# tyshiwo1/Accelerating-T2I-AR-with-SJD

Measured on AMD Instinct MI355X. Metric: accepted image-tokens/s (SJD, Lumina-mGPT-7B 768px); tokens_per_step = 1/steps-to-converge rate, higher is better.
Workload: dtype bf16; 1 GPU; Lumina-mGPT-7B 768x768, 1 prompt/GPU, draft window 16, CFG 3.0 (batch 2), top-k 2000, bf16, random-init synthetic weights (embed_token_scale=0.7); prompt_len=64, kv_len_start=401, kv_len_end=2064, lead_in_steps=131, prompts=1, parallelism=prompt-parallel x1

## Files before the change

### accelerating-t2i-ar-with-sjd_amd/_lib.py

```python
import ctypes
import os

MAX_WINDOW = 64
MAX_RANGES = 4
DTYPE_BF16, DTYPE_F16, DTYPE_F32 = 0, 1, 2
F1_POST_NORM = 0x100
F2_ROPE_TABLE = 0x200
QKN_SHARDS_SHIFT = 16

_HERE = os.path.dirname(os.path.abspath(__file__))
SO_PATH = os.environ.get("SJD_HIP_LIB") or os.path.join(_HERE, "libsjd_hip.so")


class RowRule(ctypes.Structure):
    _fields_ = [("n_ranges", ctypes.c_int32), ("lo", ctypes.c_int32 * MAX_RANGES), ("hi", ctypes.c_int32 * MAX_RANGES),
                ("forced", ctypes.c_int32), ("top_k", ctypes.c_int32), ("top_p_thr", ctypes.c_float), ("temperature", ctypes.c_float)]


class IterParams(ctypes.Structure):
    _fields_ = [("n_rows", ctypes.c_int32), ("kv_len", ctypes.c_int32), ("use_cfg", ctypes.c_int32),
                ("scheme", ctypes.c_int32), ("n_fresh", ctypes.c_int32), ("batch_rows", ctypes.c_int32), ("iter_seq", ctypes.c_int32), ("philox_blocks", ctypes.c_int32),
                ("philox_seed", ctypes.c_uint64), ("philox_offset", ctypes.c_uint64 * 3),
                ("fresh_tok", ctypes.c_int64 * MAX_WINDOW), ("rules", RowRule * MAX_WINDOW),
                ("resid_rules", RowRule * MAX_WINDOW)]


class State(ctypes.Structure):
    _fields_ = [("m", ctypes.c_int32), ("rejected", ctypes.c_int32), ("n_prev", ctypes.c_int32),
                ("prob_buf", ctypes.c_int32), ("tokens", ctypes.c_int64 * MAX_WINDOW),
                ("win_tok", ctypes.c_int64 * MAX_WINDOW), ("q_src", ctypes.c_int32 * MAX_WINDOW), ("amax", ctypes.c_int64 * MAX_WINDOW)]


class RowNorm(ctypes.Structure):
    _fields_ = [("sumsq", ctypes.c_void_p), ("slices", ctypes.c_int32), ("hidden", ctypes.c_int32), ("eps", ctypes.c_float)]


class Slots(ctypes.Structure):
    _fields_ = [("n_slots", ctypes.c_int32), ("head_rows", ctypes.c_int32), ("params_stride", ctypes.c_int64), ("state_stride", ctypes.c_int64),
                ("probs_stride", ctypes.c_int64), ("zero_state_stride", ctypes.c_int64), ("scratch_stride", ctypes.c_int64),
                ("mirror_stride", ctypes.c_int64), ("dbg_stride", ctypes.c_int64)]


class HeadPartials(ctypes.Structure):
    _fields_ = [("part", ctypes.c_void_p), ("n_chunks", ctypes.c_int32), ("chunk_stride", ctypes.c_int64), ("row_stride", ctypes.c_int64),
                ("col0", ctypes.c_int32), ("n_cols", ctypes.c_int32), ("urow_off", ctypes.c_int32), ("round_dtype", ctypes.c_int32),
                ("row_sumsq", ctypes.c_void_p), ("slices", ctypes.c_int32), ("prows", ctypes.c_int32), ("inv_hidden", ctypes.c_float),
                ("eps", ctypes.c_float), ("dbg_c", ctypes.c_void_p), ("dbg_u", ctypes.c_void_p), ("zero_state", ctypes.c_void_p)]


class L2Head(ctypes.Structure):
    _fields_ = [("wz", ctypes.c_void_p), ("kind", ctypes.c_int32), ("gx", ctypes.c_int32), ("gy", ctypes.c_int32), ("waves", ctypes.c_int32),
                ("n_tiles", ctypes.c_int32), ("tile0", ctypes.c_int32), ("n_out", ctypes.c_int32), ("pairs_full", ctypes.c_int32),
                ("pairs_last", ctypes.c_int32), ("step_major", ctypes.c_int32), ("head_pairs", ctypes.c_int32)]


EXPORTS = ["sjd_version", "sjd_error_string", "sjd_reguess", "sjd_logits_to_probs_sample", "sjd_verify_accept",
           "sjd_kv_append", "sjd_attention_workspace_bytes", "sjd_draft_window_attention", "sjd_draft_window_attention_ex",
# ... 135 lines not shown
```

### accelerating-t2i-ar-with-sjd_amd/backbones.py

```python
import math
from dataclasses import dataclass
from typing import Optional

import torch
import torch.nn as nn
import torch.nn.functional as F


import logging as _logging
import os as _os
_log = _logging.getLogger("sjd_amd.backbones")

_K1_FUSED_DEFAULT = _os.environ.get("SJD_K1_FUSED", "0") == "1"
_K1_FUSED_SPLIT_DEFAULT = _os.environ.get("SJD_K1_FUSED_SPLIT", "1") != "0"
_MLP_PAIR_DEFAULT = _os.environ.get("SJD_MLP_PAIR", "0") == "1"
_NAN_CHECK = _os.environ.get("SJD_NAN_CHECK", "0") == "1"


def _chk(tag, x, rows=None):
    if not _NAN_CHECK or x is None:
        return x
    t = x.data if hasattr(x, "n_chunks") else x
    v = t if rows is None else (t[:, :rows] if hasattr(x, "n_chunks") else t[:rows])
    if not torch.isfinite(v.float()).all():
# ... 590 lines not shown
        self.buffers_version = getattr(self, "buffers_version", 0) + 1
        return scales

    def _f2(self, qkv, li, qn, pos, B, n, params, kv_len, row_norm=None):
        ops, H, Hkv, D = self._ops, self.n_heads, self.n_kv_heads, self.head_dim
        return ops.qknorm_rope_append(qkv, self.cache.k[li], self.cache.v[li], *qn, self._inv_freq32, pos, B, n, H, Hkv, D, params,
                                      kv_len if params is None else 0, kv_scale=self.attn.scale_of(li) if hasattr(self.attn, "scale_of") else (1.0, 1.0),
                                      dtype=self.lm_head.weight.dtype, row_norm=row_norm, qk_shards=self.args.model_parallel_size)

    def _attention_block(self, qkv_part, li, qn, pos, B, n, params, kv_len, key_start, row_norm=None):
        ops, H, Hkv, D = self._ops, self.n_heads, self.n_kv_heads, self.head_dim
        ks_ok = isinstance(key_start, torch.Tensor) and key_start.is_cuda and key_start.dtype == torch.int32
        if getattr(self, "k1_fused", _K1_FUSED_DEFAULT) and ks_ok and not self.args.swin_norm and self.args.model_parallel_size == 1 and ops.fused_attention_ok(B, n, H, Hkv, D, self.cache.k.dtype):
            ns, ws = 1, None
            if getattr(self, "k1_fused_split", _K1_FUSED_SPLIT_DEFAULT):
                ns = self.attn._resolve_split(B, Hkv, n, H)
                ws = self.attn._workspace(B, H, n, D, self.cache.k.device) if ns > 1 else None
            return ops.qkv_attention_fused(qkv_part, self.cache.k[li], self.cache.v[li], *qn, self._inv_freq32, pos, B, n, H, D, params,
                                           kv_len if params is None else 0, key_start, row_norm=row_norm, dtype=self.lm_head.weight.dtype,
                                           n_split=ns, workspace=ws)
        q = self._f2(qkv_part, li, qn, pos, B, n, params, kv_len, row_norm=row_norm)
        return self.attn.attend(li, q, self.cache, kv_len, key_start)

    def _forward_window_g1_folded(self, tokens, positions, kv_len, key_start, cols=None, head_partials=False):
        ops, B, n = self._ops, tokens.shape[0], tokens.shape[1]
        T, eps, cfg = B * n, self.args.rms_norm_eps, self.G1_CFG
        self._prefetch_plan()
        g1 = lambda x_, name, N_, K_: self._g1(li, x_, name, N_, K_)
        H, Hkv, D, hid, inter = self.n_heads, self.n_kv_heads, self.head_dim, self.args.hidden_size, self.args.intermediate_size
        params = getattr(self.attn, "params", None)
        want_fused = getattr(self, "gateup_fused", _GATEUP_FUSED_DEFAULT)
        fuse_mlp = want_fused and (T <= 64 or want_fused == "tall") and not self._pf_on and ops.gateup_silu_ok(T, inter, hid, cfg["gate_up"][0],
                                                                                                                   isinstance(self._packed[0]["gate_up"], ops.PackedZ))
        red = getattr(self, "reduce_fused", _REDUCE_FUSED_DEFAULT) and not self._pf_on
        raw = lambda name: not isinstance(self._packed[0][name], ops.PackedZ)
        h_dev = self.lm_head.weight.device
        red_o = red and raw("o") and ops.skinny_gemm_reduce_ok(T, hid, H * D, cfg["o"][0], 8, h_dev)
        red_d = red and raw("down") and ops.skinny_gemm_reduce_ok(T, hid, inter, cfg["down"][0], 8, h_dev)
        pair_mlp = (getattr(self, "mlp_pair", _MLP_PAIR_DEFAULT) and fuse_mlp and not red_d and h_dev.type == "cuda" and
                    ops.mlp_pair_ok(T, inter, hid, self._packed[0]["gate_up"], self._packed[0]["down"], cfg["down"][0], cfg["down"][1], h_dev))
        h = self.model.embed_tokens(tokens).view(T, -1).contiguous()
        pos = positions.reshape(T).contiguous()
        delta, ss_next = None, None
        for li, layer in enumerate(self.model.layers):
            a = layer.self_attn
            rn = (ss_next if ss_next is not None else ops.residual_sumsq(h, delta), hid, eps)
            qn = (a.q_norm.weight, a.q_norm.bias, a.k_norm.weight, a.k_norm.bias) if self.args.qk_norm else (None,) * 4
            _chk(f"L{li} sumsq", rn[0][:, :T] if rn[0].dim() == 2 and rn[0].shape[1] >= T else rn[0])
            o = self._attention_block(_chk(f"L{li} qkv", g1(h, "qkv", (H + 2 * Hkv) * D, hid), T), li, qn, pos, B, n, params, kv_len, key_start, row_norm=rn)
            _chk(f"L{li} attention", o)
            if red_o:
                rn = (ops.skinny_gemm_reduce(o.view(T, H * D), self._packed[li]["o"], hid, H * D, cfg["o"][0], h, 8, cfg["o"][2]), hid, eps)
            else:
                rn = (ops.residual_sumsq(h, g1(o.view(T, H * D), "o", hid, H * D)), hid, eps)
            if pair_mlp:
                if getattr(self, "_pair_ready", None) is None or self._pair_ready.device != h.device:
                    self._pair_ready = torch.zeros(max(64, (inter + cfg["down"][0] - 1) // cfg["down"][0] + 1), dtype=torch.int32, device=h.device)
                _, delta = ops.mlp_pair(h, self._packed[li]["gate_up"], self._packed[li]["down"], inter, hid, cfg["down"][0], row_norm=rn,
                                        ready=self._pair_ready)
                ss_next = None
                continue
            if fuse_mlp:
                act = ops.gateup_silu(h, self._packed[li]["gate_up"], inter, hid, cfg["gate_up"][2], row_norm=rn)
            else:
                act = ops.silu_mul(g1(h, "gate_up", 2 * inter, hid), rows=T, dtype=h.dtype, row_norm=rn)
            _chk(f"L{li} act", act)
# ... 25 lines not shown
        pos = positions.reshape(T).contiguous()
        delta = None
        swin = self.args.swin_norm
        for li, layer in enumerate(self.model.layers):
            a = layer.self_attn
            x = h if swin else ops.add_rmsnorm(h, delta, layer.input_layernorm.weight, eps)
            qkv = g1(x, "qkv", (H + 2 * Hkv) * D, hid)
            qn = (a.q_norm.weight, a.q_norm.bias, a.k_norm.weight, a.k_norm.bias) if self.args.qk_norm else (None,) * 4
            o = self._attention_block(qkv, li, qn, pos, B, n, params, kv_len, key_start)
            attn_out = g1(o.view(T, H * D), "o", hid, H * D)
            if swin:
                x = ops.add_rmsnorm_post(h, attn_out, layer.input_layernorm.weight, eps)
            else:
                x = ops.add_rmsnorm(h, attn_out, layer.post_attention_layernorm.weight, eps)
            gu = g1(x, "gate_up", 2 * inter, hid)
            act = ops.silu_mul(gu, rows=T, dtype=h.dtype)
            delta = g1(act, "down", hid, inter)
            if swin:
                ops.add_rmsnorm_post(h, delta, layer.post_attention_layernorm.weight, eps)
                delta = None
        x = ops.add_rmsnorm(h, delta, self.model.norm.weight, eps)
        return _head_logits(self.lm_head, x, cols).view(B, n, -1)

    def _forward_window_fused(self, tokens, positions, kv_len, key_start, cols=None, head_partials=False):
        T_ = tokens.shape[0] * tokens.shape[1]
        if self._gemm == "sjd" and (T_ <= 64 or (T_ <= 128 and tokens.shape[1] <= 32) or
                                    (T_ <= 256 and tokens.shape[1] <= 32 and self._packed and not isinstance(self._packed[0]["qkv"], self._ops.PackedZ)
                                     and all(c[1] in self.G1_WIDE_TILES for c in self.G1_CFG.values()))):
            if self._fold_norm:
                return self._forward_window_g1_folded(tokens, positions, kv_len, key_start, cols, head_partials)
            return self._forward_window_g1(tokens, positions, kv_len, key_start, cols)
        ops, B, n = self._ops, tokens.shape[0], tokens.shape[1]
        T, eps = B * n, self.args.rms_norm_eps
        H, Hkv, D = self.n_heads, self.n_kv_heads, self.head_dim
        params = getattr(self.attn, "params", None)
        h = self.model.embed_tokens(tokens).view(T, -1).contiguous()
        pos = positions.reshape(T).contiguous()
        delta = None
        swin = self.args.swin_norm
        for li, layer in enumerate(self.model.layers):
            a = layer.self_attn
            qkv_w, gu_w = self._fused[li]
            x = h if swin else ops.add_rmsnorm(h, delta, layer.input_layernorm.weight, eps)
            qkv = F.linear(x, qkv_w)
            qn = (a.q_norm.weight, a.q_norm.bias, a.k_norm.weight, a.k_norm.bias) if self.args.qk_norm else (None,) * 4
            q = _chk(f"prefill L{li} q", self._f2(_chk(f"prefill L{li} qkv", qkv), li, qn, pos, B, n, params, kv_len))
            o = _chk(f"prefill L{li} attention", self.attn.attend(li, q, self.cache, kv_len, key_start))
            attn_out = F.linear(o.view(T, H * D), a.o_proj.weight)
            if swin:
                x = _chk(f"prefill L{li} norm1", ops.add_rmsnorm_post(h, attn_out, layer.input_layernorm.weight, eps))
                ops.add_rmsnorm_post(h, _chk(f"prefill L{li} mlp", F.linear(ops.silu_mul(F.linear(x, gu_w)), layer.mlp.down_proj.weight)),
                                     layer.post_attention_layernorm.weight, eps)
                continue
            x = _chk(f"prefill L{li} norm2", ops.add_rmsnorm(h, attn_out, layer.post_attention_layernorm.weight, eps))
            delta = _chk(f"prefill L{li} mlp", F.linear(ops.silu_mul(F.linear(x, gu_w)), layer.mlp.down_proj.weight))
        x = ops.add_rmsnorm(h, delta, self.model.norm.weight, eps)
        return _head_logits(self.lm_head, x, cols).view(B, n, -1)

    def forward_window(self, tokens, positions, kv_len, key_start, cols=None, head_partials=False):
        if getattr(self, "_ops", None) is not None:
            return self._forward_window_fused(tokens, positions, kv_len, key_start, cols, head_partials)
        B, n = tokens.shape
        h = self.model.embed_tokens(tokens)
        cos, sin = self._rope(positions, h.dtype)
        for li, layer in enumerate(self.model.layers):
            a = layer.self_attn
            x = h if self.args.swin_norm else layer.input_layernorm(h)
            q = a.q_proj(x).view(B, n, a.num_heads, a.head_dim)
            k = a.k_proj(x).view(B, n, a.num_kv, a.head_dim)
            v = a.v_proj(x).view(B, n, a.num_kv, a.head_dim)
            if self.args.qk_norm:
                q, k = a.q_norm(q), a.k_norm(k)
            q = q * cos + _rotate_half(q) * sin
            k = k * cos + _rotate_half(k) * sin
            o = self.attn(li, q, k, v, self.cache, kv_len, key_start)
            if self.args.swin_norm:
                h = h + layer.input_layernorm(a.o_proj(o.reshape(B, n, -1)))
                h = h + layer.post_attention_layernorm(layer.mlp(h))
                continue
            h = h + a.o_proj(o.reshape(B, n, -1))
            h = h + layer.mlp(layer.post_attention_layernorm(h))
        return _head_logits(self.lm_head, self.model.norm(h), cols)


# ... 8 lines not shown
```

### accelerating-t2i-ar-with-sjd_amd/csrc/sjd_glue.hip

```cpp
#include <hip/hip_runtime.h>
#include <math.h>

#include "../../include/sjd_hip.h"

#ifdef SJD_TRACE
__device__ unsigned long long g_glue_trace[3][4096][4];
#define SJD_TRG(k, i) do { if (threadIdx.x == 0) g_glue_trace[k][((blockIdx.y * gridDim.x) + blockIdx.x) & 4095][i] = wall_clock64(); } while (0)
extern "C" int sjd_debug_trace_glue(int kind, unsigned long long *host_out, int n_wg)
{
    return hipMemcpyFromSymbol(host_out, HIP_SYMBOL(g_glue_trace), (size_t)n_wg * 4 * sizeof(unsigned long long),
                               (size_t)kind * 4096 * 4 * sizeof(unsigned long long), hipMemcpyDeviceToHost) == hipSuccess ? 0 : -1;
}
#else
#define SJD_TRG(k, i) do { } while (0)
#endif

typedef __attribute__((ext_vector_type(4))) unsigned u32x4;

#include "sjd_mlp_epilogue.h"
#ifdef SJD_EXPERIMENTAL
#include "sjd_l2_prefetch.h"
#endif

template <int DT> struct Cvt;
template <> struct Cvt<SJD_DTYPE_BF16> {
    static __device__ __forceinline__ float to_f(unsigned short h) { return __uint_as_float((unsigned)h << 16); }
    static __device__ __forceinline__ unsigned short from_f(float x)
    {
        unsigned u = __float_as_uint(x);
        u += 0x7fffu + ((u >> 16) & 1u);
        return (unsigned short)(u >> 16);
    }
};
template <> struct Cvt<SJD_DTYPE_F16> {
    static __device__ __forceinline__ float to_f(unsigned short h) { return (float)(*reinterpret_cast<_Float16 *>(&h)); }
    static __device__ __forceinline__ unsigned short from_f(float x)
    {
        _Float16 h = (_Float16)x;
        return *reinterpret_cast<unsigned short *>(&h);
    }
};

// ... 225 lines not shown
            for (int j = 0; j < 4; ++j) {
                o[j] = sjd_residual_elem<DT>(hx[j], dd[j]);
                hx[j] = Cvt<DT>::to_f(o[j]);
            }
            uint2 ho;
            ho.x = (unsigned)o[0] | ((unsigned)o[1] << 16);
            ho.y = (unsigned)o[2] | ((unsigned)o[3] << 16);
            *reinterpret_cast<uint2 *>(hp) = ho;
        }
        ss = sjd_sumsq4(ss, hx[0], hx[1], hx[2], hx[3]);
    }
    ss = wave_sum(ss);
    if ((threadIdx.x & 63) == 0) red[threadIdx.x >> 6] = ss;
    __syncthreads();
    if (threadIdx.x == 0) out_sumsq[(size_t)blockIdx.y * prows + row] = red[0] + red[1];
    SJD_TRG(0, 2);
}

template <int DT>
__global__ __launch_bounds__(128) void f1r_residual_sumsq(unsigned short *__restrict__ h, const float *__restrict__ part, int n_chunks,
                                                          int hidden, int prows, float *__restrict__ out_sumsq)
{
    f1r_body<DT>(h, part, n_chunks, hidden, prows, out_sumsq);
}

#ifdef SJD_EXPERIMENTAL
template <int DT>
__global__ __launch_bounds__(128) void f1r_residual_sumsq_pf(unsigned short *__restrict__ h, const float *__restrict__ part, int n_chunks,
                                                             int hidden, int prows, float *__restrict__ out_sumsq, int n_slices,
                                                             const sjd_l2_head pf)
{
    if ((int)blockIdx.y >= n_slices) {
        sjd_l2_head_pull(pf, ((int)blockIdx.y - n_slices) * (int)gridDim.x + (int)blockIdx.x, ((int)gridDim.y - n_slices) * (int)gridDim.x);
        return;
    }
    f1r_body<DT>(h, part, n_chunks, hidden, prows, out_sumsq);
}

#endif
__device__ __forceinline__ float row_sumsq_total(const float *__restrict__ row_sumsq, int slices, int prows, int row)
{
    float t = 0.f;
    for (int s0 = 0; s0 < slices; s0 += 8) {
        float v[8];
#pragma unroll
        for (int q = 0; q < 8; ++q) v[q] = (s0 + q < slices) ? row_sumsq[(size_t)(s0 + q) * prows + row] : 0.f;
// ... 554 lines not shown
}

extern "C" int sjd_qknorm_rope_append_fp8(const void *qkv, void *q_out, void *k_cache, void *v_cache, const void *qn_w, const void *qn_b,
                                          const void *kn_w, const void *kn_b, const float *inv_freq, const int64_t *positions, int B, int n,
                                          int H, int H_kv, int D, int S_max, int dtype, float k_scale, float v_scale,
                                          const sjd_iter_params *params, int kv_len, const float *part, int n_chunks, void *stream)
{
    return f2_launch(qkv, q_out, k_cache, v_cache, qn_w, qn_b, kn_w, kn_b, inv_freq, positions, B, n, H, H_kv, D, S_max, dtype, params, kv_len,
                     part, n_chunks, true, k_scale, v_scale, nullptr, stream);
}

extern "C" int sjd_qknorm_rope_append_ex(const void *qkv, void *q_out, void *k_cache, void *v_cache, const void *qn_w, const void *qn_b,
                                         const void *kn_w, const void *kn_b, const float *inv_freq, const int64_t *positions, int B, int n,
                                         int H, int H_kv, int D, int S_max, int dtype, int kv_fp8, float k_scale, float v_scale,
                                         const sjd_row_norm *row_norm, const sjd_iter_params *params, int kv_len, const float *part,
                                         int n_chunks, void *stream)
{
    return f2_launch(qkv, q_out, k_cache, v_cache, qn_w, qn_b, kn_w, kn_b, inv_freq, positions, B, n, H, H_kv, D, S_max, dtype, params, kv_len,
                     part, n_chunks, kv_fp8 != 0, k_scale, v_scale, row_norm, stream);
}

extern "C" int sjd_residual_sumsq(void *h, const float *part, int n_chunks, int rows, int hidden, int dtype, float *out_sumsq, void *stream)
{
    if (!h || !out_sumsq || rows < 1 || rows > 256 || (part && n_chunks < 1) || hidden < 4 || (hidden % 4) != 0) return SJD_ERR_BAD_ARG;
    const int prows = ((rows + 31) / 32) * 32;
    const dim3 grid(rows, (hidden + 511) / 512), block(128);
    hipStream_t s = (hipStream_t)stream;
    if (dtype == SJD_DTYPE_BF16)
        hipLaunchKernelGGL(f1r_residual_sumsq<SJD_DTYPE_BF16>, grid, block, 0, s, (unsigned short *)h, part, n_chunks, hidden, prows, out_sumsq);
    else if (dtype == SJD_DTYPE_F16)
        hipLaunchKernelGGL(f1r_residual_sumsq<SJD_DTYPE_F16>, grid, block, 0, s, (unsigned short *)h, part, n_chunks, hidden, prows, out_sumsq);
    else return SJD_ERR_UNSUPPORTED;
    return hipGetLastError() == hipSuccess ? SJD_OK : SJD_ERR_LAUNCH;
}

#ifdef SJD_EXPERIMENTAL
extern "C" int sjd_residual_sumsq_pf(void *h, const float *part, int n_chunks, int rows, int hidden, int dtype, float *out_sumsq,
                                     const sjd_l2_head *head, int pf_blocks, void *stream)
{
    if (!head || pf_blocks < 1) return sjd_residual_sumsq(h, part, n_chunks, rows, hidden, dtype, out_sumsq, stream);
    if (!h || !out_sumsq || rows < 1 || rows > 256 || (part && n_chunks < 1) || hidden < 4 || (hidden % 4) != 0 || !head->wz) return SJD_ERR_BAD_ARG;
    const int prows = ((rows + 31) / 32) * 32, n_slices = (hidden + 511) / 512;
    int pf_rows = (pf_blocks + rows - 1) / rows;
    while ((pf_rows * rows) % 8) ++pf_rows;
    if ((rows * n_slices) % 8) return sjd_residual_sumsq(h, part, n_chunks, rows, hidden, dtype, out_sumsq, stream);
    const dim3 grid(rows, n_slices + pf_rows), block(128);
// ... 43 lines not shown
```

### accelerating-t2i-ar-with-sjd_amd/csrc/sjd_sampling.hip

```cpp
#include <hip/hip_runtime.h>
#include <math.h>
#include <type_traits>

#include "../../include/sjd_hip.h"
#include "sjd_device.h"
#include "sjd_philox.h"

#ifdef SJD_TRACE
__device__ unsigned long long g_k2_trace[64][16];
#define SJD_TRS(slot, i) do { if (threadIdx.x == 0) g_k2_trace[(slot) & 63][i] = wall_clock64(); } while (0)
extern "C" int sjd_debug_trace_k2(unsigned long long *host_out, int n)
{
    return hipMemcpyFromSymbol(host_out, HIP_SYMBOL(g_k2_trace), (size_t)n * 16 * sizeof(unsigned long long), 0, hipMemcpyDeviceToHost) == hipSuccess ? 0 : -1;
}
#else
#define SJD_TRS(slot, i) do { } while (0)
#endif

__device__ __forceinline__ void rule_window(const sjd_row_rule &r, int V, int &lo, int &hi)
{
    if (r.n_ranges == 0) { lo = 0; hi = V; return; }
    lo = V; hi = 0;
#pragma unroll
    for (int a = 0; a < SJD_MAX_RANGES; ++a)
        if (a < r.n_ranges) { lo = min(lo, r.lo[a]); hi = max(hi, r.hi[a]); }
    lo = max(lo, 0); hi = min(hi, V);
    if (hi < lo) hi = lo;
}

// ... 744 lines not shown
            if (res_lds) resample(std::true_type{}); else resample(std::false_type{});
        }
    }
    if (threadIdx.x == 0) { state->m = m; state->rejected = rejected ? (degenerate ? 2 : 1) : 0; state->n_prev = n; }
    SJD_TRS(32, 5);
    k4_mirror_state(state, host_mirror, params->iter_seq);
    SJD_TRS(32, 6);
}

template <bool SLOTS = false>
__global__ void k5_reguess(const sjd_iter_params *__restrict__ params, sjd_state *__restrict__ state,
                           int64_t *__restrict__ input_ids_out, int n_batch, int max_rows, const int64_t *__restrict__ pos_offset,
                           int64_t *__restrict__ positions_out, const sjd_slots sb)
{
    if constexpr (SLOTS) {
        const size_t s = blockIdx.x;
        params = reinterpret_cast<const sjd_iter_params *>(reinterpret_cast<const char *>(params) + s * (size_t)sb.params_stride);
        state = reinterpret_cast<sjd_state *>(reinterpret_cast<char *>(state) + s * (size_t)sb.state_stride);
        input_ids_out += s * (size_t)n_batch * (size_t)max_rows;
        if (pos_offset) pos_offset += s * (size_t)n_batch;
        if (positions_out) positions_out += s * (size_t)n_batch * (size_t)max_rows;
    }
    const int i = threadIdx.x;
    const int n = params->n_rows;
    const int m = state->m, n_prev = state->n_prev;
    int a = n_prev - m;
    if (a > n - 1) a = n - 1;
    if (a < 0) a = 0;
    int64_t tok = 0;
    int qs = -1;
    if (i < n) {
        if (i <= a) { tok = state->tokens[m - 1 + i]; qs = m - 1 + i; }
        else { tok = params->fresh_tok[i - 1 - a]; qs = -1; }
    }
    __syncthreads();
    if (i < max_rows) {
        if (i >= n) { tok = state->tokens[m - 1]; qs = -1; }
        state->win_tok[i] = tok;
        state->q_src[i] = qs;
        for (int b = 0; b < n_batch; ++b) input_ids_out[(size_t)b * max_rows + i] = tok;
        if (positions_out) {
            const int64_t base = (int64_t)params->kv_len + i;
            for (int b = 0; b < n_batch; ++b) positions_out[(size_t)b * max_rows + i] = base + (pos_offset ? pos_offset[b] : 0);
        }
    }
}

#define SJD_DRAW_LIST 2304
static int sjd_stage_lds_floats(long cols)
{
    const long cap = 150 * 1024 / 4;
    return (int)(cols < cap ? ((cols + 3) & ~3L) : cap);
}

extern "C" int sjd_reguess_ex(const sjd_iter_params *params, sjd_state *state, int64_t *input_ids_out, int n_batch, int max_rows,
                              const int64_t *pos_offset, int64_t *positions_out, void *stream)
{
    if (!params || !state || !input_ids_out || max_rows < 1 || max_rows > SJD_MAX_WINDOW || n_batch < 1) return SJD_ERR_BAD_ARG;
    hipLaunchKernelGGL(k5_reguess<false>, dim3(1), dim3(64), 0, (hipStream_t)stream, params, state, input_ids_out, n_batch, max_rows, pos_offset,
                       positions_out, sjd_slots{});
// ... 144 lines not shown
```

### accelerating-t2i-ar-with-sjd_amd/engine.py

```python
import contextlib
import ctypes
import gc
import os
import random
import time
import warnings
from dataclasses import dataclass, field
from typing import List, Optional

import numpy as np
import torch

from . import _lib as L
from . import ops
from .grammar import spatial_fresh_tokens


_MIRROR_STREAM_WAIT = os.environ.get("SJD_MIRROR_SPIN", "0") != "1"
_TWO_STAGE = os.environ.get("SJD_TWO_STAGE", "0") == "1"


@dataclass
class SJDConfig:
    jacobi_loop_interval_l: int = 1
# ... 97 lines not shown
        self.backbone, self.V, self.device, self.Lmax, self.B = backbone, int(vocab_size), torch.device(device), max_window, n_batch
        dev = self.device
        self.params = ops.DeviceBlob(L.IterParams, dev)
        self.state = ops.DeviceBlob(L.State, dev)
        self.probs = torch.zeros(2, self.Lmax, self.V, dtype=torch.float32, device=dev)
        self.zero_state = torch.full((2, self.Lmax, 2), -1, dtype=torch.int32, device=dev)
        self.noise = self.rs = self.noise2 = None
        self._philox = True
        self.scratch = torch.empty(self.V, dtype=torch.float32, device=dev)
        self.input_ids = torch.zeros(self.B, self.Lmax, dtype=torch.int64, device=dev)
        self.arange = torch.arange(self.Lmax, device=dev)
        self.positions = torch.zeros(self.B, self.Lmax, dtype=torch.int64, device=dev)
        self.tokens_ptr = self.state.field_ptr("tokens")
        self.amax_ptr = self.state.field_ptr("amax")
        self.key_start = torch.zeros(self.B, dtype=torch.int32, device=dev)
        self.pos_offset = torch.zeros(self.B, dtype=torch.int64, device=dev)
        off = L.IterParams.kv_len.offset
        self.kv_len_dev = self.params.dev[off:off + 4].view(torch.int32)
        self.hook = None
        self.use_graph = use_graph
        self.narrow_head = narrow_head
        self.head_partials = bool(head_partials) and getattr(backbone, "supports_head_partials", False)
        self._dbg = None
        self._guidance = 3.0
        self._rule_bytes, self._rule_keep, self._cols_cache = {}, [], {}
        self._seq = 0
        self.reset_graphs()

    def reset_graphs(self):
        self._graphs, self._graph_logits, self._eager_runs = {}, {}, {}
        self.__dict__.pop("_graph_sig", None)

    def _check_graph_buffers(self):
        attn = getattr(self.backbone, "attn", None)
        cache = getattr(self.backbone, "cache", None)
        sig = (getattr(attn, "ws_version", 0), getattr(self.backbone, "buffers_version", 0),
               cache.k.data_ptr() if cache is not None else 0, cache.v.data_ptr() if cache is not None else 0)
        if sig != getattr(self, "_graph_sig", sig):
            self.reset_graphs()
        self._graph_sig = sig

    def _noise_tensors(self):
        if self.noise is None:
            dev = self.device
            self.noise = torch.ones(self.Lmax, self.V, dtype=torch.float32, device=dev)
            self.rs = torch.zeros(self.Lmax, self.V, dtype=torch.float32, device=dev)
# ... 14 lines not shown
            p.fresh_tok[:len(fresh)] = fresh
        self._write_rules(L.IterParams.rules.offset, rules)
        if resid:
            self._write_rules(L.IterParams.resid_rules.offset, resid)
        self.params.upload(L.IterParams.resid_rules.offset if head_only else None)

    def _write_rules(self, offset, rules):
        key = tuple(map(id, rules))
        blk = self._rule_bytes.get(key)
        if blk is None:
            blk = b"".join(bytes(r) for r in rules)
            if len(self._rule_bytes) < 4096:
                self._rule_bytes[key] = blk
                self._rule_keep.append(list(rules))
        ctypes.memmove(self.params.host.data_ptr() + offset, blk, len(blk))

    def _upload_resid(self, resid):
        off = L.IterParams.resid_rules.offset
        self._write_rules(off, resid)
        L.check(L.load().sjd_upload_async(self.params.dev.data_ptr() + off, self.params.host.data_ptr() + off, self.params.nbytes - off,
                                          ops._stream()), "sjd_upload_async")

    def _forward_body(self, cols=None):
        ops.reguess(self.params, self.state, self.input_ids, pos_offset=self.pos_offset, positions_out=self.positions)
        positions = self.positions
        if self.head_partials:
            return self.backbone.forward_window(self.input_ids, positions, -1, self.key_start, cols=cols, head_partials=True)
        if cols is None:
            return self.backbone.forward_window(self.input_ids, positions, -1, self.key_start)
        return self.backbone.forward_window(self.input_ids, positions, -1, self.key_start, cols=cols)

    def _calibrate_fp8(self, tokens, positions, key_start):
        bb = self.backbone
        cache, attn = getattr(bb, "cache", None), getattr(bb, "attn", None)
        if (cache is None or cache.k.dtype != ops.FP8 or attn is None or getattr(attn, "layer_scales", 1) is not None
                or getattr(attn, "kv_scale", (1.0, 1.0)) != (1.0, 1.0) or not hasattr(bb, "calibrate_kv_scales")
                or os.environ.get("SJD_FP8_CALIBRATE", "1") == "0"):
            return
        bb.calibrate_kv_scales(tokens, positions, key_start)

    def _k2_out(self):
        return (self.amax_ptr, self.tokens_ptr) if getattr(self, "_greedy", False) else (self.tokens_ptr, self.amax_ptr)

    def _sample_body(self, cur, logits, cols=None):
        noise, rs, noise2 = (None, None, None) if self._philox else (self.noise, self.rs, self.noise2[0])
        if isinstance(logits, ops.HeadOut):
# ... 328 lines not shown
```

### accelerating-t2i-ar-with-sjd_amd/ops.py

```python
import ctypes
import os

import torch

from . import _lib as L


def _stream():
    return ctypes.c_void_p(torch.cuda.current_stream().cuda_stream)


def _ptr(t):
    return ctypes.c_void_p(0 if t is None else t.data_ptr())


def _dtype_code(dt):
    if dt == torch.bfloat16:
        return L.DTYPE_BF16
    if dt == torch.float16:
        return L.DTYPE_F16
    if dt == torch.float32:
        return L.DTYPE_F32
    raise L.SjdLibraryError(f"SJD HIP kernels support bf16/fp16 KV and activations, got {dt}")

# ... 113 lines not shown
        self.host.copy_(self.dev)

    def wait_mirror(self):
        L.check(L.load().sjd_stream_synchronize(_stream()), "sjd_stream_synchronize")
        for b in self.blobs:
            if b._mirror is not None:
                b.collect_mirror()

    @property
    def ptr(self):
        return ctypes.c_void_p(self.dev.data_ptr())


def reguess(params: DeviceBlob, state: DeviceBlob, input_ids_out: torch.Tensor, pos_offset=None, positions_out=None):
    n_batch, max_rows = input_ids_out.shape
    assert input_ids_out.dtype == torch.int64 and input_ids_out.is_contiguous()
    if positions_out is None:
        L.check(L.load().sjd_reguess(params.ptr, state.ptr, _ptr(input_ids_out), n_batch, max_rows, _stream()), "sjd_reguess")
        return
    assert positions_out.dtype == torch.int64 and positions_out.is_contiguous() and tuple(positions_out.shape) == (n_batch, max_rows)
    assert pos_offset is None or (pos_offset.dtype == torch.int64 and pos_offset.is_contiguous() and pos_offset.numel() == n_batch)
    L.check(L.load().sjd_reguess_ex(params.ptr, state.ptr, _ptr(input_ids_out), n_batch, max_rows, _ptr(pos_offset) if pos_offset is not None else None,
                                   _ptr(positions_out), _stream()), "sjd_reguess_ex")


def logits_to_probs_sample(logits_c, logits_u, guidance, params: DeviceBlob, noise, probs_out, tokens_out_ptr, col0=0, amax_out_ptr=None):
    max_rows, V = probs_out.shape
    assert logits_c.dtype == torch.float32 and logits_c.stride(-1) == 1 and probs_out.is_contiguous()
    assert noise is None or (noise.dtype == torch.float32 and noise.is_contiguous() and noise.shape[-1] == V)
    if logits_u is not None:
        assert logits_u.stride(-2) == logits_c.stride(-2) and logits_u.stride(-1) == 1
    shift = lambda t: ctypes.c_void_p(0 if t is None else t.data_ptr() - 4 * int(col0))
    L.check(L.load().sjd_logits_to_probs_sample_ex(shift(logits_c), shift(logits_u), logits_c.stride(-2), float(guidance),
                                                  max_rows, V, params.ptr, _ptr(noise), _ptr(probs_out), tokens_out_ptr, amax_out_ptr,
                                                  _stream()), "sjd_logits_to_probs_sample")


def verify_accept(params: DeviceBlob, state: DeviceBlob, probs, prev_probs, rs, noise2, scratch, mirror=False):
    max_rows, V = probs.shape
    for t in (probs, prev_probs, rs, noise2, scratch):
        assert t is None or (t.dtype == torch.float32 and t.is_contiguous())
    L.check(L.load().sjd_verify_accept_ex(params.ptr, state.ptr, _ptr(probs), _ptr(prev_probs), _ptr(rs), _ptr(noise2),
                                         _ptr(scratch), max_rows, V, state.mirror_ptr if mirror else None, _stream()), "sjd_verify_accept")


def kv_append(k_new, v_new, k_cache, v_cache, params, kv_len):
# ... 810 lines not shown
```

### include/sjd_hip.h

```cpp
#ifndef SJD_HIP_H
#define SJD_HIP_H

#include <stdint.h>

#ifdef __cplusplus
extern "C" {
#endif

#define SJD_VERSION 103
#define SJD_MAX_WINDOW 64
#define SJD_MAX_RANGES 4

#define SJD_OK 0
#define SJD_ERR_BAD_ARG (-1)
#define SJD_ERR_UNSUPPORTED (-2)
#define SJD_ERR_LAUNCH (-3)

#define SJD_DTYPE_BF16 0
#define SJD_DTYPE_F16 1
#define SJD_DTYPE_F32 2

#define SJD_DTYPE_MASK 0xff
#define SJD_F1_POST_NORM 0x100
#define SJD_F2_ROPE_TABLE 0x200
#define SJD_QKN_SHARDS_SHIFT 16
#define SJD_QKN_SHARDS_MASK (0xff << SJD_QKN_SHARDS_SHIFT)
#define SJD_QKN_SHARDS(mp) ((int)(mp) << SJD_QKN_SHARDS_SHIFT)

typedef struct sjd_row_rule {
    int32_t n_ranges;
    int32_t lo[SJD_MAX_RANGES];
    int32_t hi[SJD_MAX_RANGES];
    int32_t forced;
    int32_t top_k;
    float   top_p_thr;
    float   temperature;
} sjd_row_rule;

typedef struct sjd_iter_params {
    int32_t n_rows;
    int32_t kv_len;
    int32_t use_cfg;
    int32_t scheme;
    int32_t n_fresh;
    int32_t batch_rows;
    int32_t iter_seq;
    int32_t philox_blocks;
// ... 105 lines not shown
                               int H, int H_kv, int D, int S_max, int dtype, const int32_t *key_start,
                               const sjd_iter_params *params, int kv_len, int n_split, void *workspace, void *stream);

int sjd_draft_window_attention_ex(const void *q, const void *k_cache, const void *v_cache, void *out, int B, int n_rows,
                                  int H, int H_kv, int D, int S_max, int dtype, const int32_t *key_start,
                                  const sjd_iter_params *params, int kv_len, int n_split, void *workspace, void *stream,
                                  void *ev_start, void *ev_stop);



int sjd_add_rmsnorm(void *h, const void *delta, const void *weight, void *y, int rows, int hidden, float eps, int dtype,
                    const float *part, int n_chunks, void *stream);
int sjd_qknorm_rope_append(const void *qkv, void *q_out, void *k_cache, void *v_cache, const void *qn_w, const void *qn_b,
                           const void *kn_w, const void *kn_b, const float *inv_freq, const int64_t *positions, int B, int n,
                           int H, int H_kv, int D, int S_max, int dtype, const sjd_iter_params *params, int kv_len,
                           const float *part, int n_chunks, void *stream);
int sjd_silu_mul(const void *gate_up, void *y, int rows, int inter, int dtype, const float *part, int n_chunks, void *stream);

typedef struct sjd_row_norm {
    const float *sumsq;
    int32_t slices, hidden;
    float eps;
} sjd_row_norm;
int sjd_residual_sumsq(void *h, const float *part, int n_chunks, int rows, int hidden, int dtype, float *out_sumsq, void *stream);
int sjd_qknorm_rope_append_ex(const void *qkv, void *q_out, void *k_cache, void *v_cache, const void *qn_w, const void *qn_b,
                              const void *kn_w, const void *kn_b, const float *inv_freq, const int64_t *positions, int B, int n,
                              int H, int H_kv, int D, int S_max, int dtype, int kv_fp8, float k_scale, float v_scale,
                              const sjd_row_norm *row_norm, const sjd_iter_params *params, int kv_len, const float *part,
                              int n_chunks, void *stream);
int sjd_silu_mul_ex(const void *gate_up, void *y, int rows, int inter, int dtype, const float *part, int n_chunks,
                    const sjd_row_norm *row_norm, void *stream);

int sjd_gateup_silu(const void *x, const void *w_packed, void *y, int M, int I, int K, int step_major, int dtype,
                    const sjd_row_norm *row_norm, void *stream);

int sjd_gemm_num_chunks(int K, int KC);

int sjd_skinny_gemm_cols(const void *x, const void *w_packed, float *out, int M, int N, int K, int KC, int waves, int step_major,
                         int dtype, int N_packed, int tile0, void *stream);
int sjd_skinny_gemm(const void *x, const void *w_packed, float *out, int M, int N, int K, int KC, int waves, int step_major,
                    int dtype, void *stream);

int sjd_skinny_gemm_z(const void *x, const void *wz, const void *exc, int exc_cap, float *out, int M, int N, int K, int KC, int waves, int step_major,
                      int dtype, int N_packed, int tile0, void *stream);
int sjd_gateup_silu_z(const void *x, const void *wz, const void *exc, int exc_cap, void *y, int M, int I, int K, int step_major, int dtype,
                      const sjd_row_norm *row_norm, void *stream);
// ... 47 lines not shown
```

Before: 772.6 image-tokens/s.

## Fuse reguess, embedding gather and first-layer sumsq into one front kernel

Adds a front kernel that recomputes the window tokens (the reguess step), writes input ids and positions, gathers embedding rows into the hidden buffer and computes the per-row sum of squares for the first layer's folded RMSNorm, all in one launch. The folded G1 window path takes this precomputed (h, sumsq) instead of running reguess, embedding lookup and residual_sumsq as separate launches. It removes two kernel launches and one extra pass over h per window step. In exchange, the token selection is recomputed in every block, and state is written by the first column block of each batch-0 row.

```diff
diff --git a/accelerating-t2i-ar-with-sjd_amd/_lib.py b/accelerating-t2i-ar-with-sjd_amd/_lib.py
--- a/accelerating-t2i-ar-with-sjd_amd/_lib.py
+++ b/accelerating-t2i-ar-with-sjd_amd/_lib.py
@@ -6,6 +6,7 @@
 DTYPE_BF16, DTYPE_F16, DTYPE_F32 = 0, 1, 2
 F1_POST_NORM = 0x100
 F2_ROPE_TABLE = 0x200
+F1R_FRONT = 0x400
 QKN_SHARDS_SHIFT = 16
 
 _HERE = os.path.dirname(os.path.abspath(__file__))
@@ -33,6 +34,12 @@
 
 class RowNorm(ctypes.Structure):
     _fields_ = [("sumsq", ctypes.c_void_p), ("slices", ctypes.c_int32), ("hidden", ctypes.c_int32), ("eps", ctypes.c_float)]
+
+
+class Front(ctypes.Structure):
+    _fields_ = [("params", ctypes.c_void_p), ("state", ctypes.c_void_p), ("input_ids_out", ctypes.c_void_p), ("pos_offset", ctypes.c_void_p),
+                ("positions_out", ctypes.c_void_p), ("embed", ctypes.c_void_p), ("vocab", ctypes.c_int32), ("n_batch", ctypes.c_int32),
+                ("max_rows", ctypes.c_int32), ("reserved", ctypes.c_int32)]
 
 
 class Slots(ctypes.Structure):
diff --git a/accelerating-t2i-ar-with-sjd_amd/backbones.py b/accelerating-t2i-ar-with-sjd_amd/backbones.py
--- a/accelerating-t2i-ar-with-sjd_amd/backbones.py
+++ b/accelerating-t2i-ar-with-sjd_amd/backbones.py
@@ -636,7 +636,7 @@
         q = self._f2(qkv_part, li, qn, pos, B, n, params, kv_len, row_norm=row_norm)
         return self.attn.attend(li, q, self.cache, kv_len, key_start)
 
-    def _forward_window_g1_folded(self, tokens, positions, kv_len, key_start, cols=None, head_partials=False):
+    def _forward_window_g1_folded(self, tokens, positions, kv_len, key_start, cols=None, head_partials=False, front=None):
         ops, B, n = self._ops, tokens.shape[0], tokens.shape[1]
         T, eps, cfg = B * n, self.args.rms_norm_eps, self.G1_CFG
         self._prefetch_plan()
@@ -653,9 +653,15 @@
         red_d = red and raw("down") and ops.skinny_gemm_reduce_ok(T, hid, inter, cfg["down"][0], 8, h_dev)
         pair_mlp = (getattr(self, "mlp_pair", _MLP_PAIR_DEFAULT) and fuse_mlp and not red_d and h_dev.type == "cuda" and
                     ops.mlp_pair_ok(T, inter, hid, self._packed[0]["gate_up"], self._packed[0]["down"], cfg["down"][0], cfg["down"][1], h_dev))
-        h = self.model.embed_tokens(tokens).view(T, -1).contiguous()
+        if front is not None:
+            h, ss_next = front
+            if tuple(h.shape) != (T, hid) or h.dtype != self.lm_head.weight.dtype or not h.is_contiguous():
+                raise ValueError(f"front: h {tuple(h.shape)} {h.dtype} does not fit a {T}-row window of this backbone")
+            delta = None
+        else:
+            h = self.model.embed_tokens(tokens).view(T, -1).contiguous()
+            delta, ss_next = None, None
         pos = positions.reshape(T).contiguous()
-        delta, ss_next = None, None
         for li, layer in enumerate(self.model.layers):
             a = layer.self_attn
             rn = (ss_next if ss_next is not None else ops.residual_sumsq(h, delta), hid, eps)
@@ -727,14 +733,29 @@
         x = ops.add_rmsnorm(h, delta, self.model.norm.weight, eps)
         return _head_logits(self.lm_head, x, cols).view(B, n, -1)
 
-    def _forward_window_fused(self, tokens, positions, kv_len, key_start, cols=None, head_partials=False):
-        T_ = tokens.shape[0] * tokens.shape[1]
-        if self._gemm == "sjd" and (T_ <= 64 or (T_ <= 128 and tokens.shape[1] <= 32) or
-                                    (T_ <= 256 and tokens.shape[1] <= 32 and self._packed and not isinstance(self._packed[0]["qkv"], self._ops.PackedZ)
-                                     and all(c[1] in self.G1_WIDE_TILES for c in self.G1_CFG.values()))):
+    def _window_on_g1(self, B, n):
+        T_ = B * n
+        return self._gemm == "sjd" and (T_ <= 64 or (T_ <= 128 and n <= 32) or
+                                        (T_ <= 256 and n <= 32 and self._packed and not isinstance(self._packed[0]["qkv"], self._ops.PackedZ)
+                                         and all(c[1] in self.G1_WIDE_TILES for c in self.G1_CFG.values())))
+
+    def window_front(self, B, n):
+        if getattr(self, "_ops", None) is None or not self._window_on_g1(B, n) or not self._fold_norm:
+            return None
+        w = self.model.embed_tokens.weight
+        ok = (w.dtype in (torch.bfloat16, torch.float16) and w.dtype == self.lm_head.weight.dtype and w.is_contiguous() and w.is_cuda
+              and w.shape[1] % 4 == 0)
+        return w if ok else None
+
+    def _forward_window_fused(self, tokens, positions, kv_len, key_start, cols=None, head_partials=False, front=None):
+        if self._window_on_g1(tokens.shape[0], tokens.shape[1]):
             if self._fold_norm:
-                return self._forward_window_g1_folded(tokens, positions, kv_len, key_start, cols, head_partials)
+                return self._forward_window_g1_folded(tokens, positions, kv_len, key_start, cols, head_partials, front=front)
+            if front is not None:
+                raise ValueError("front: only the folded G1 window path takes a precomputed (h, sumsq) -- ask window_front() first")
             return self._forward_window_g1(tokens, positions, kv_len, key_start, cols)
+        if front is not None:
+            raise ValueError("front: only the folded G1 window path takes a precomputed (h, sumsq) -- ask window_front() first")
         ops, B, n = self._ops, tokens.shape[0], tokens.shape[1]
         T, eps = B * n, self.args.rms_norm_eps
         H, Hkv, D = self.n_heads, self.n_kv_heads, self.head_dim
@@ -762,9 +783,11 @@
         x = ops.add_rmsnorm(h, delta, self.model.norm.weight, eps)
         return _head_logits(self.lm_head, x, cols).view(B, n, -1)
 
-    def forward_window(self, tokens, positions, kv_len, key_start, cols=None, head_partials=False):
+    def forward_window(self, tokens, positions, kv_len, key_start, cols=None, head_partials=False, front=None):
         if getattr(self, "_ops", None) is not None:
-            return self._forward_window_fused(tokens, positions, kv_len, key_start, cols, head_partials)
+            return self._forward_window_fused(tokens, positions, kv_len, key_start, cols, head_partials, front=front)
+        if front is not None:
+            raise ValueError("front: only the folded G1 window path takes a precomputed (h, sumsq) -- ask window_front() first")
         B, n = tokens.shape
         h = self.model.embed_tokens(tokens)
         cos, sin = self._rope(positions, h.dtype)
diff --git a/accelerating-t2i-ar-with-sjd_amd/csrc/sjd_glue.hip b/accelerating-t2i-ar-with-sjd_amd/csrc/sjd_glue.hip
--- a/accelerating-t2i-ar-with-sjd_amd/csrc/sjd_glue.hip
+++ b/accelerating-t2i-ar-with-sjd_amd/csrc/sjd_glue.hip
@@ -18,6 +18,7 @@
 typedef __attribute__((ext_vector_type(4))) unsigned u32x4;
 
 #include "sjd_mlp_epilogue.h"
+#include "sjd_reguess.h"
 #ifdef SJD_EXPERIMENTAL
 #include "sjd_l2_prefetch.h"
 #endif
@@ -289,6 +290,36 @@
                                                           int hidden, int prows, float *__restrict__ out_sumsq)
 {
     f1r_body<DT>(h, part, n_chunks, hidden, prows, out_sumsq);
+}
+
+template <int DT>
+__global__ __launch_bounds__(128) void f1r_front(const sjd_front f, unsigned short *__restrict__ h, int hidden, int prows,
+                                                 float *__restrict__ out_sumsq)
+{
+    __shared__ float red[2];
+    const int row = blockIdx.x, c = blockIdx.y * 512 + threadIdx.x * 4;
+    const int b = row / f.max_rows, i = row - b * f.max_rows;
+    int64_t tok;
+    int qs;
+    sjd_k5_row(f.params, f.state, i, tok, qs);
+    if (blockIdx.y == 0 && threadIdx.x == 0) {
+        if (b == 0) { f.state->win_tok[i] = tok; f.state->q_src[i] = qs; }
+        f.input_ids_out[row] = tok;
+        if (f.positions_out) f.positions_out[row] = (int64_t)f.params->kv_len + i + (f.pos_offset ? f.pos_offset[b] : 0);
+    }
+    const int64_t trow = tok < 0 ? 0 : (tok >= (int64_t)f.vocab ? (int64_t)f.vocab - 1 : tok);
+    float ss = 0.f;
+    if (c < hidden) {
+        const uint2 hv = *reinterpret_cast<const uint2 *>(reinterpret_cast<const unsigned short *>(f.embed) + (size_t)trow * hidden + c);
+        *reinterpret_cast<uint2 *>(h + (size_t)row * hidden + c) = hv;
+        const float hx[4] = {Cvt<DT>::to_f((unsigned short)(hv.x & 0xffffu)), Cvt<DT>::to_f((unsigned short)(hv.x >> 16)),
+                             Cvt<DT>::to_f((unsigned short)(hv.y & 0xffffu)), Cvt<DT>::to_f((unsigned short)(hv.y >> 16))};
+        ss = sjd_sumsq4(ss, hx[0], hx[1], hx[2], hx[3]);
+    }
+    ss = wave_sum(ss);
+    if ((threadIdx.x & 63) == 0) red[threadIdx.x >> 6] = ss;
+    __syncthreads();
+    if (threadIdx.x == 0) out_sumsq[(size_t)blockIdx.y * prows + row] = red[0] + red[1];
 }
 
 #ifdef SJD_EXPERIMENTAL
@@ -889,6 +920,23 @@
 
 extern "C" int sjd_residual_sumsq(void *h, const float *part, int n_chunks, int rows, int hidden, int dtype, float *out_sumsq, void *stream)
 {
+    if (dtype & ~(SJD_DTYPE_MASK | SJD_F1R_FRONT)) return SJD_ERR_UNSUPPORTED;
+    if (dtype & SJD_F1R_FRONT) {
+        const sjd_front *f = reinterpret_cast<const sjd_front *>(part);
+        dtype &= SJD_DTYPE_MASK;
+        if (!h || !out_sumsq || !f || n_chunks != 0 || rows < 1 || rows > 256 || hidden < 4 || (hidden % 4) != 0) return SJD_ERR_BAD_ARG;
+        if (!f->params || !f->state || !f->input_ids_out || !f->embed || f->vocab < 1 || f->n_batch < 1 || f->max_rows < 1 ||
+            f->max_rows > SJD_MAX_WINDOW || (int64_t)f->n_batch * f->max_rows != rows) return SJD_ERR_BAD_ARG;
+        if (((uintptr_t)h & 7) || ((uintptr_t)f->embed & 7)) return SJD_ERR_BAD_ARG;
+        const int prows_f = ((rows + 31) / 32) * 32;
+        const dim3 grid_f(rows, (hidden + 511) / 512), block_f(128);
+        if (dtype == SJD_DTYPE_BF16)
+            hipLaunchKernelGGL(f1r_front<SJD_DTYPE_BF16>, grid_f, block_f, 0, (hipStream_t)stream, *f, (unsigned short *)h, hidden, prows_f, out_sumsq);
+        else if (dtype == SJD_DTYPE_F16)
+            hipLaunchKernelGGL(f1r_front<SJD_DTYPE_F16>, grid_f, block_f, 0, (hipStream_t)stream, *f, (unsigned short *)h, hidden, prows_f, out_sumsq);
+        else return SJD_ERR_UNSUPPORTED;
+        return hipGetLastError() == hipSuccess ? SJD_OK : SJD_ERR_LAUNCH;
+    }
     if (!h || !out_sumsq || rows < 1 || rows > 256 || (part && n_chunks < 1) || hidden < 4 || (hidden % 4) != 0) return SJD_ERR_BAD_ARG;
     const int prows = ((rows + 31) / 32) * 32;
     const dim3 grid(rows, (hidden + 511) / 512), block(128);
diff --git a/accelerating-t2i-ar-with-sjd_amd/csrc/sjd_reguess.h b/accelerating-t2i-ar-with-sjd_amd/csrc/sjd_reguess.h
--- /dev/null
+++ b/accelerating-t2i-ar-with-sjd_amd/csrc/sjd_reguess.h
@@ -0,0 +1,19 @@
+#pragma once
+#include <stdint.h>
+
+#include "../../include/sjd_hip.h"
+
+__device__ __forceinline__ void sjd_k5_row(const sjd_iter_params *params, const sjd_state *state, int i, int64_t &tok, int &qs)
+{
+    const int n = params->n_rows;
+    const int m = state->m, n_prev = state->n_prev;
+    int a = n_prev - m;
+    if (a > n - 1) a = n - 1;
+    if (a < 0) a = 0;
+    tok = 0;
+    qs = -1;
+    if (i < n) {
+        if (i <= a) { tok = state->tokens[m - 1 + i]; qs = m - 1 + i; }
+        else { tok = params->fresh_tok[i - 1 - a]; qs = -1; }
+    } else { tok = state->tokens[m - 1]; qs = -1; }
+}
diff --git a/accelerating-t2i-ar-with-sjd_amd/csrc/sjd_sampling.hip b/accelerating-t2i-ar-with-sjd_amd/csrc/sjd_sampling.hip
--- a/accelerating-t2i-ar-with-sjd_amd/csrc/sjd_sampling.hip
+++ b/accelerating-t2i-ar-with-sjd_amd/csrc/sjd_sampling.hip
@@ -5,6 +5,7 @@
 #include "../../include/sjd_hip.h"
 #include "sjd_device.h"
 #include "sjd_philox.h"
+#include "sjd_reguess.h"
 
 #ifdef SJD_TRACE
 __device__ unsigned long long g_k2_trace[64][16];
@@ -795,20 +796,11 @@
         if (positions_out) positions_out += s * (size_t)n_batch * (size_t)max_rows;
     }
     const int i = threadIdx.x;
-    const int n = params->n_rows;
-    const int m = state->m, n_prev = state->n_prev;
-    int a = n_prev - m;
-    if (a > n - 1) a = n - 1;
-    if (a < 0) a = 0;
     int64_t tok = 0;
     int qs = -1;
-    if (i < n) {
-        if (i <= a) { tok = state->tokens[m - 1 + i]; qs = m - 1 + i; }
-        else { tok = params->fresh_tok[i - 1 - a]; qs = -1; }
-    }
+    if (i < max_rows) sjd_k5_row(params, state, i, tok, qs);
     __syncthreads();
     if (i < max_rows) {
-        if (i >= n) { tok = state->tokens[m - 1]; qs = -1; }
         state->win_tok[i] = tok;
         state->q_src[i] = qs;
         for (int b = 0; b < n_batch; ++b) input_ids_out[(size_t)b * max_rows + i] = tok;
diff --git a/accelerating-t2i-ar-with-sjd_amd/engine.py b/accelerating-t2i-ar-with-sjd_amd/engine.py
--- a/accelerating-t2i-ar-with-sjd_amd/engine.py
+++ b/accelerating-t2i-ar-with-sjd_amd/engine.py
@@ -143,6 +143,7 @@
         self.narrow_head = narrow_head
         self.head_partials = bool(head_partials) and getattr(backbone, "supports_head_partials", False)
         self._dbg = None
+        self.fused_front = True
         self._guidance = 3.0
         self._rule_bytes, self._rule_keep, self._cols_cache = {}, [], {}
         self._seq = 0
@@ -203,6 +204,14 @@
                                           ops._stream()), "sjd_upload_async")
 
     def _forward_body(self, cols=None):
+        wf = getattr(self.backbone, "window_front", None)
+        embed = wf(self.B, self.Lmax) if (wf is not None and self.fused_front) else None
+        if embed is not None:
+            front = ops.reguess_embed_sumsq(self.params, self.state, self.input_ids, embed, pos_offset=self.pos_offset, positions_out=self.positions)
+            kw = {"cols": cols} if cols is not None else {}
+            if self.head_partials:
+                kw["head_partials"] = True
+            return self.backbone.forward_window(self.input_ids, self.positions, -1, self.key_start, front=front, **kw)
         ops.reguess(self.params, self.state, self.input_ids, pos_offset=self.pos_offset, positions_out=self.positions)
         positions = self.positions
         if self.head_partials:
diff --git a/accelerating-t2i-ar-with-sjd_amd/ops.py b/accelerating-t2i-ar-with-sjd_amd/ops.py
--- a/accelerating-t2i-ar-with-sjd_amd/ops.py
+++ b/accelerating-t2i-ar-with-sjd_amd/ops.py
@@ -159,6 +159,25 @@
     assert pos_offset is None or (pos_offset.dtype == torch.int64 and pos_offset.is_contiguous() and pos_offset.numel() == n_batch)
     L.check(L.load().sjd_reguess_ex(params.ptr, state.ptr, _ptr(input_ids_out), n_batch, max_rows, _ptr(pos_offset) if pos_offset is not None else None,
                                    _ptr(positions_out), _stream()), "sjd_reguess_ex")
+
+
+def reguess_embed_sumsq(params: DeviceBlob, state: DeviceBlob, input_ids_out: torch.Tensor, embed: torch.Tensor, pos_offset=None, positions_out=None):
+    n_batch, max_rows = input_ids_out.shape
+    assert input_ids_out.dtype == torch.int64 and input_ids_out.is_contiguous()
+    assert embed.dim() == 2 and embed.is_contiguous() and embed.device == input_ids_out.device, "embed: a contiguous [vocab, hidden] table on the ids' device"
+    assert positions_out is None or (positions_out.dtype == torch.int64 and positions_out.is_contiguous() and tuple(positions_out.shape) == (n_batch, max_rows))
+    assert pos_offset is None or (pos_offset.dtype == torch.int64 and pos_offset.is_contiguous() and pos_offset.numel() == n_batch)
+    vocab, hidden = embed.shape
+    T = n_batch * max_rows
+    if T > 256 or hidden % 4:
+        raise ValueError(f"reguess_embed_sumsq: {T} rows x {hidden} columns (at most 256 rows, hidden a multiple of 4)")
+    h = torch.empty(T, hidden, dtype=embed.dtype, device=embed.device)
+    out = torch.empty((hidden + 511) // 512, _prows(T), dtype=torch.float32, device=embed.device)
+    f = L.Front(params.ptr.value, state.ptr.value, input_ids_out.data_ptr(), pos_offset.data_ptr() if pos_offset is not None else None,
+                positions_out.data_ptr() if positions_out is not None else None, embed.data_ptr(), vocab, n_batch, max_rows, 0)
+    L.check(L.load().sjd_residual_sumsq(_ptr(h), ctypes.cast(ctypes.pointer(f), ctypes.c_void_p), 0, T, hidden, _dtype_code(embed.dtype) | L.F1R_FRONT,
+                                       _ptr(out), _stream()), "sjd_residual_sumsq (front)")
+    return h, out
 
 
 def logits_to_probs_sample(logits_c, logits_u, guidance, params: DeviceBlob, noise, probs_out, tokens_out_ptr, col0=0, amax_out_ptr=None):
diff --git a/include/sjd_hip.h b/include/sjd_hip.h
--- a/include/sjd_hip.h
+++ b/include/sjd_hip.h
@@ -23,6 +23,7 @@
 #define SJD_DTYPE_MASK 0xff
 #define SJD_F1_POST_NORM 0x100
 #define SJD_F2_ROPE_TABLE 0x200
+#define SJD_F1R_FRONT 0x400
 #define SJD_QKN_SHARDS_SHIFT 16
 #define SJD_QKN_SHARDS_MASK (0xff << SJD_QKN_SHARDS_SHIFT)
 #define SJD_QKN_SHARDS(mp) ((int)(mp) << SJD_QKN_SHARDS_SHIFT)
@@ -174,6 +175,15 @@
     int32_t slices, hidden;
     float eps;
 } sjd_row_norm;
+typedef struct sjd_front {
+    const sjd_iter_params *params;
+    sjd_state *state;
+    int64_t *input_ids_out;
+    const int64_t *pos_offset;
+    int64_t *positions_out;
+    const void *embed;
+    int32_t vocab, n_batch, max_rows, reserved;
+} sjd_front;
 int sjd_residual_sumsq(void *h, const float *part, int n_chunks, int rows, int hidden, int dtype, float *out_sumsq, void *stream);
 int sjd_qknorm_rope_append_ex(const void *qkv, void *q_out, void *k_cache, void *v_cache, const void *qn_w, const void *qn_b,
                               const void *kn_w, const void *kn_b, const float *inv_freq, const int64_t *positions, int B, int n,
```

Measured after the change: 773.8 image-tokens/s (median of 2 runs). Within noise of the previous version (+0.2%).
